# Tung-I/Dual-awareness-Attention-for-Few-shot-Object-Detection

Hardware: AMD Instinct MI355X
Metric: query-images/sec (res50, way=2, shot=3, bs=4 per GPU, train-mode forward) (higher is better)
Workload: dtype f32 (operands, accumulation, results; multiplies as an exact bf16x3 split, six bf16 MFMA products each)

## Files before the change

dual-awareness-attention-for-few-shot-object-detection_amd/csrc/igemm.hip:

```cpp
#include "common.h"
#include "../../include/dana_hip_debug.h"
#include <stdlib.h>
#include <atomic>

namespace {

typedef float f32x16 __attribute__((ext_vector_type(16)));
typedef unsigned int u32x4 __attribute__((ext_vector_type(4)));

struct IgemmParams {
  const float* A;
  const float* Bw;
  float* C;
  const float* scale;
  const float* shift;
  const float* residual;
  const float* mask;
  long ldm;
  int M, N, K;
  int IH, IW, OH, OW, Cin, KH, KW, stride, pad;
  int M0, IH1, IW1, OH1, OW1, pix1;
  float* C1;
  const float* residual1;
  long ldc1, ldr1;
  int lda, ldb;
  long ldc, ldr;
  long batch_a, batch_b, batch_c;
  unsigned a_bytes, b_bytes;
  float alpha;
  int relu;
  int vec_io;
  int vec_ss;
  int tiles_m, tiles_n;
  const float* A2;
  int lda2, IH2, IW2, stride2, K1;
  int IH21, IW21, pix21;
  int bpre;
  const void* Bw2;
  const float* scale2;
  const float* shift2;
  int N2, relu2;
  unsigned a2_bytes;
  int apre, a_rows;
  int res_sample, res_h, res_w, res_oh, res_ow;
  unsigned res_bytes;
  unsigned long long* trace;
};

constexpr int BK = 32;
constexpr int LDS_LD = 36;
constexpr unsigned OOB = 0x80000000u;

__device__ __forceinline__ int xcd_remap(int bid, int nwg) {
  const int q = nwg / 8, r = nwg % 8;
  const int xcd = bid % 8, local = bid / 8;
  return (xcd < r ? xcd * (q + 1) : r * (q + 1) + (xcd - r) * q) + local;
}

__device__ __forceinline__ float4 ldg_b128(__amdgpu_buffer_rsrc_t r, unsigned off) {
  u32x4 v = __builtin_amdgcn_raw_buffer_load_b128(r, (int)off, 0, 0);
  return *(float4*)&v;
}

template <int BM, int BN, int STEM>
__global__ void __launch_bounds__(256, 2) igemm_f32_kernel(IgemmParams p) {
  constexpr int TM = BM / 64, TN = BN / 64;
  constexpr int RA = BM / 32, RB = BN / 32;
  constexpr int CLD = BN + 4;
  extern __shared__ __attribute__((aligned(16))) float smem[];
  float* As = smem;
  float* Bs = smem + 2 * BM * LDS_LD;

  const int tid = threadIdx.x;
  const int lane = tid & 63, wave = tid >> 6;
  const int wm = wave >> 1, wn = wave & 1;
  const int li = lane & 31, lh = lane >> 5;

  const int vid = xcd_remap((int)(blockIdx.z * gridDim.x + blockIdx.x), (int)(gridDim.x * gridDim.z));
  const int zb = vid / (int)gridDim.x;
  const int tile = vid - zb * (int)gridDim.x;
// ... 398 lines not shown
  const int lane = tid & 63, wave = tid >> 6;
  const int wm = wave >> 1, wn = wave & 1;
  const int li = lane & 31, lh = lane >> 5;

  const unsigned long long t_start = p.trace ? __builtin_readcyclecounter() : 0ull;
  const unsigned long long w_start = p.trace ? wall_clock64() : 0ull;
  const int vid = xcd_remap((int)(blockIdx.z * gridDim.x + blockIdx.x), (int)(gridDim.x * gridDim.z));
  const int zb = vid / (int)gridDim.x;
  const int tile = vid - zb * (int)gridDim.x;
  const int tm_idx = tile / p.tiles_n, tn_idx = tile % p.tiles_n;
  const int m0 = tm_idx * BM, n0 = tn_idx * BN;
  const float* Ab = p.A + (long)zb * p.batch_a;
  const float* Bb = p.Bw + (long)zb * p.batch_b;
  float* Cb = p.C + (long)zb * p.batch_c;
  __amdgpu_buffer_rsrc_t ra_src = __builtin_amdgcn_make_buffer_rsrc((void*)Ab, 0, (int)p.a_bytes, 0x00020000);
  const __amdgpu_buffer_rsrc_t rb_src = __builtin_amdgcn_make_buffer_rsrc((void*)Bb, 0, (int)p.b_bytes, 0x00020000);

  int cin_t = STEM ? SBK : p.Cin;
  const int kw_t = STEM ? 2 : p.KW;
  const int kh_t = STEM ? 7 : p.KH;
  const int lda4 = (STEM ? 4 : p.lda) * 4;
  const int kwstep = STEM ? 4 * lda4 : lda4;
  const int c4 = tid & 3;
  const int r0 = tid >> 2;
  const int wcol = ((c4 >> 1) ^ swz(r0)) * 4 + (c4 & 1) * 2;
  const int rcol = (lh ^ swz(li)) * 4;
  const int klim = p.K - c4 * 4;
  constexpr int DEAD = (int)0x80000000;
  unsigned a_off[RA];
  unsigned a_mask[RA];
  int a_dseg[RA];
  unsigned a_off2[RA];
  const bool lin = !STEM && p.KH * p.KW == 1 && p.stride == 1 && p.pad == 0;
#pragma unroll
  for (int j = 0; j < RA; ++j) {
    const int m = m0 + r0 + 64 * j;
    const bool ok = m < p.M;
    const bool s1 = ok && m >= p.M0;
    const int mm = ok ? (s1 ? m - p.M0 : m) : 0;
    if (lin && !p.A2) {
      a_off[j] = (unsigned)(((s1 ? p.pix1 : 0) + mm) * lda4 + c4 * 16);
      a_mask[j] = ok ? 1u : 0u;
      a_dseg[j] = 0;
      a_off2[j] = OOB;
      continue;
    }
    const int IH = s1 ? p.IH1 : p.IH, IW = s1 ? p.IW1 : p.IW, OW = s1 ? p.OW1 : p.OW;
    const int ohw = (s1 ? p.OH1 : p.OH) * OW;
    const int img = mm / ohw, rem = mm - img * ohw;
    const int oh = rem / OW, ow = rem - oh * OW;
    const int ih0 = oh * p.stride - p.pad, iw0 = ow * p.stride - p.pad;
    const int pix = (s1 ? p.pix1 : 0) + (img * IH + ih0) * IW;
    unsigned mask = 0;
    if (STEM) {
      const int lo = ih0 < 0 ? -ih0 : 0, hi = IH - ih0 < 7 ? IH - ih0 : 7;
      const int iwa = iw0 + c4, iwb = iw0 + 4 + c4;
      const unsigned cv = ((iwa >= 0 && iwa < IW) ? 0x1555u : 0u) | ((iwb >= 0 && iwb < IW && c4 < 3) ? 0x2aaau : 0u);
      if (ok && hi > lo) mask = ((1u << (2 * hi)) - (1u << (2 * lo))) & cv;
    } else if (ok) {
      unsigned colbits = 0;
      for (int kw = 0; kw < kw_t; ++kw)
        if (iw0 + kw >= 0 && iw0 + kw < IW) colbits |= 1u << kw;
      for (int kh = 0; kh < kh_t; ++kh)
        if (ih0 + kh >= 0 && ih0 + kh < IH) mask |= colbits << (kh * kw_t);
    }
    a_off[j] = STEM ? (unsigned)((pix + iw0 + c4) * lda4) : (unsigned)((pix + iw0) * lda4 + c4 * 16);
    a_mask[j] = mask;
    a_dseg[j] = s1 ? (p.IW1 - p.IW) * lda4 : 0;
    a_off2[j] = (!STEM && p.A2 && ok)
                    ? (unsigned)(((s1 ? p.pix21 : 0) + ((long)img * (s1 ? p.IH21 : p.IH2) + oh * p.stride2) * (s1 ? p.IW21 : p.IW2) +
                                  ow * p.stride2) * p.lda2 * 4 + c4 * 16)
                    : OOB;
  }
  unsigned b_cur[RB];
  int b_lim[RB];
  int b_lds[RB];
#pragma unroll
  for (int j = 0; j < RB; ++j) {
    if constexpr (BPRE) {
      const int q = (tid + 256 * j < 6 * BN) ? tid + 256 * j : tid;
      const int pl = q / (2 * BN), rem = q - pl * (2 * BN);
      const int row = rem >> 1, half = rem & 1;
      const int n = n0 + row;
      b_cur[j] = (unsigned)((((long)pl * p.N + n) * SBK + half * 8) * 2);
      b_lim[j] = n < p.N ? (p.K + SBK - 1) / SBK * SBK : DEAD;
      b_lds[j] = (pl * BN + row) * SLD + (half ^ swz(row)) * 4;
    } else {
      const int n = n0 + r0 + 64 * j;
      b_cur[j] = (unsigned)((n * p.ldb + c4 * 4) * 4);
      b_lim[j] = n < p.N ? klim : DEAD;
      b_lds[j] = 0;
    }
  }
  const unsigned B_STEP = BPRE ? (unsigned)p.N * 3u * SBK * 2u : SBK * 4;

  float4 ra0[RA], rb0[RB], ra1[RA], rb1[RB];
  int lt_k0 = 0, lt_cin = 0, lt_kh = 0, lt_kw = 0;
  unsigned lt_bit = 1u;
  unsigned a_cur[RA];
  int a_lim[RA];
#pragma unroll
  for (int j = 0; j < RA; ++j) {
    a_cur[j] = a_off[j];
    a_lim[j] = (a_mask[j] & 1u) ? klim : DEAD;
  }
  auto next_tap = [&]() {
    if (lt_cin >= cin_t) {
      lt_cin = 0;
      if (!STEM && p.A2) {
        ra_src = __builtin_amdgcn_make_buffer_rsrc((void*)p.A2, 0, (int)p.a2_bytes, 0x00020000);
        cin_t = 0x7fffffff;
#pragma unroll
        for (int j = 0; j < RA; ++j) {
          a_cur[j] = a_off2[j];
          a_lim[j] = a_off2[j] != OOB ? klim : DEAD;
        }
        return;
      }
// ... 180 lines not shown
            asm volatile("" : "+v"(lb[f][e0]), "+v"(lb[f][e1]));
          } else if constexpr (r == 8) {
            hp[f].x = __builtin_amdgcn_perm(hb[f][1], hb[f][0], 0x07060302u);
            hp[f].y = __builtin_amdgcn_perm(hb[f][3], hb[f][2], 0x07060302u);
            asm volatile("" : "+v"(hp[f].x), "+v"(hp[f].y));
          } else if constexpr (r == 9) {
            mp[f].x = __builtin_amdgcn_perm(mb[f][1], mb[f][0], 0x07060302u);
            mp[f].y = __builtin_amdgcn_perm(mb[f][3], mb[f][2], 0x07060302u);
            asm volatile("" : "+v"(mp[f].x), "+v"(mp[f].y));
          } else if constexpr (r == 10) {
            lp[f].x = __builtin_amdgcn_perm(lb[f][1], lb[f][0], 0x07060302u);
            lp[f].y = __builtin_amdgcn_perm(lb[f][3], lb[f][2], 0x07060302u);
            asm volatile("" : "+v"(lp[f].x), "+v"(lp[f].y));
          } else {
            unsigned* w = f < RA ? aw + 64 * f * SLD : bw + 64 * (f - RA) * SLD;
            constexpr int rows = f < RA ? BM : BN;
            if constexpr (r == 11) {
              *(uint2*)(w + 0 * rows * SLD) = hp[f];
              *(uint2*)(w + 1 * rows * SLD) = mp[f];
            } else {
              *(uint2*)(w + 2 * rows * SLD) = lp[f];
            }
          }
        }
      });
      __builtin_amdgcn_sched_barrier(0);
    });
  };
  const unsigned long long t_loop = p.trace ? __builtin_readcyclecounter() : 0ull;
  for (int t = 0; t < nk; t += 2) {
    k_step(0, fa0, fb0, fa1, fb1, ra0, rb0, ra1, rb1);
    k_step(1, fa1, fb1, fa0, fb0, ra1, rb1, ra0, rb0);
  }
  if constexpr (FUSE || ELDS) __syncthreads();
  const unsigned long long t_loop_end = p.trace ? __builtin_readcyclecounter() : 0ull;

  if constexpr (FUSE) {
    static_assert(BM == 128 && BN == 64 && !STEM && BPRE, "fused tail: 128 x 64 tile over pre-split weights");
    unsigned short* A2 = (unsigned short*)smem;
    unsigned* rtab = (unsigned*)smem + 4 * 3 * BM * 16 * 2 / 4;
    if constexpr (FUSE == 2) {
      if (tid < BM) {
        const int m = m0 + tid;
        unsigned off = OOB;
        if (m < p.M) {
          const int ohw = p.OH * p.OW;
          const int img = m / ohw, rem = m - img * ohw;
          const int oh = rem / p.OW, ow = rem - oh * p.OW;
          off = (unsigned)((((long)img * p.IH + oh * p.stride) * p.IW + ow * p.stride) * p.ldr * 4);
        }
        rtab[tid] = off;
      }
    }
    {
      const int nn = wn * 32 + li;
      const float sc1 = p.scale ? p.scale[nn] : 1.f, sh1 = p.shift ? p.shift[nn] : 0.f;
      const int ks = nn >> 4, kk = nn & 15;
#pragma unroll
      for (int i = 0; i < TM; ++i)
#pragma unroll
        for (int r = 0; r < 16; ++r) {
          const int row = wm * (BM / 2) + i * 32 + (r & 3) + 8 * (r >> 2) + 4 * lh;
          float v = acc[i][0][r] * sc1 + sh1;
          if (p.relu) v = fmaxf(v, 0.f);
          const unsigned hb = __float_as_uint(v) & 0xffff0000u;
          const float r1 = v - __uint_as_float(hb);
          const unsigned mb = __float_as_uint(r1) & 0xffff0000u;
          const unsigned lb = __float_as_uint(r1 - __uint_as_float(mb));
// ... 269 lines not shown
      const bool s1 = m >= p.M0;
      float* cp = s1 ? p.C1 + (long)(m - p.M0) * p.ldc1 + n : Cb + (long)m * p.ldc + n;
      const float* rp = s1 ? p.residual1 + (long)(m - p.M0) * p.ldr1 + n : p.residual + (long)m * p.ldr + n;
      for (int t = 0; t < 4; ++t)
        if ((n + t) < p.N) {
          float x = Cs[rr * CLD + ec + t] * sc[t] + sh[t];
          if (p.residual) x += rp[t];
          if (p.relu) x = fmaxf(x, 0.f);
          if (p.mask && !(p.mask[(long)m * p.ldm + n + t] > 0.f)) x = 0.f;
          cp[t] = x;
        }
    }
  }
  if (p.trace && tid == 0) {
    unsigned long long* tr = p.trace + ((long)blockIdx.z * gridDim.x + blockIdx.x) * 8;
    tr[0] = t_start;
    tr[1] = t_loop;
    tr[2] = t_loop_end;
    tr[3] = __builtin_readcyclecounter();
    tr[4] = (unsigned long long)__builtin_amdgcn_s_getreg((31 << 11) | 4) | ((unsigned long long)__builtin_amdgcn_s_getreg((31 << 11) | 20) << 32);
    tr[5] = wall_clock64();
    tr[6] = w_start;
    tr[7] = 0;
  }
}

template <int BM, int BN, int STEM, int BPRE = 0, int FUSE = 0, int ELDS = 0, int RSMP = 0>
__global__ void __launch_bounds__(256, 2) igemm_split_kernel(IgemmParams p) {
  igemm_split_body<BM, BN, STEM, BPRE, FUSE, ELDS, RSMP>(p);
}
template <int STEM, int BPRE, int ELDS, int RSMP = 0>
__global__ void __launch_bounds__(256, 1) __attribute__((amdgpu_num_vgpr(192))) igemm_split_kernel_128(IgemmParams p) {
  igemm_split_body<128, 128, STEM, BPRE, 0, ELDS, RSMP>(p);
}

template <int BN, int NST, int APRE, int DF = 0>
__global__ void __launch_bounds__(256, NST == 2 ? 3 : (NST == 3 ? 2 : 1)) igemm_dma_kernel(IgemmParams p) {
  static_assert(APRE || NST == 2, "fp32 activation rows: two stages");
  static_assert(!DF || (APRE && NST >= 3), "two fragment sets: planes x planes, three or more stages");
  constexpr int BM = 128, TM = 2, TN = BN / 64;
  constexpr int STAGE_B = 3 * (BM + BN) * 32;
  constexpr int NPB = 3 * BN / 32, PB = (NPB + 3) / 4;
  constexpr int NDMA = (APRE ? 3 : 0) + PB;
  constexpr int AHEAD = NST == 2 ? 2 : NST - 1;
  constexpr int RA = BM / 64;
  extern __shared__ __attribute__((aligned(16))) float smem[];
  const int tid = threadIdx.x;
  const int lane = tid & 63, wave = __builtin_amdgcn_readfirstlane(tid >> 6);
  const int wm = wave >> 1, wn = wave & 1;
  const int li = lane & 31, lh = lane >> 5;
  const unsigned long long t_start = p.trace ? __builtin_readcyclecounter() : 0ull;
  const unsigned long long w_start = p.trace ? wall_clock64() : 0ull;
  const int vid = xcd_remap((int)(blockIdx.z * gridDim.x + blockIdx.x), (int)(gridDim.x * gridDim.z));
  const int zb = vid / (int)gridDim.x;
  const int tile = vid - zb * (int)gridDim.x;
  const int tm_idx = tile / p.tiles_n, tn_idx = tile % p.tiles_n;
  const int m0 = tm_idx * BM, n0 = tn_idx * BN;
  float* Cb = p.C + (long)zb * p.batch_c;
  __amdgpu_buffer_rsrc_t ra_src =
      __builtin_amdgcn_make_buffer_rsrc((void*)(p.A + (long)zb * p.batch_a), 0, (int)p.a_bytes, 0x00020000);
  const __amdgpu_buffer_rsrc_t rb_src =
      __builtin_amdgcn_make_buffer_rsrc((void*)(p.Bw + (long)zb * p.batch_b), 0, (int)p.b_bytes, 0x00020000);
  const int nk = (p.K + SBK - 1) / SBK;

  const int prow = lane >> 1, phalf = (lane & 1) ^ ((lane >> 4) & 1);
  const int arow = m0 + 32 * wave + prow;
// ... 354 lines not shown
  igemm_f32_kernel<BM, BN, STEM><<<grid, 256, lds, s>>>(p);
  return 0;
}

template <int BM, int BN, int STEM = 0, int BPRE = 0, int FUSE = 0, int ELDS = 0, int RSMP = 0>
int launch_split(const IgemmParams& p0, int batch, hipStream_t s) {
  if constexpr (BPRE == 0 && FUSE == 0) {
    if (p0.bpre) return launch_split<BM, BN, STEM, 1, 0, ELDS, RSMP>(p0, batch, s);
  }
  if constexpr (ELDS == 0 && FUSE == 0 && RSMP == 0) {
    if (epilogue_mode_cell().load(std::memory_order_relaxed)) return launch_split<BM, BN, STEM, BPRE, 0, 1>(p0, batch, s);
  }
  g_last_form.store(form_code(BM * BN >= 128 * 128 ? DANA_IGEMM_FAMILY_SPLIT_128 : DANA_IGEMM_FAMILY_SPLIT, BM, BN, STEM, BPRE, FUSE ? 1 : 0,
                              ELDS, 0, 0, 0), std::memory_order_relaxed);
  IgemmParams p = p0;
  p.tiles_m = (p.M + BM - 1) / BM;
  p.tiles_n = (p.N + BN - 1) / BN;
  size_t lds = (size_t)2 * 3 * (BM + BN) * SLD * sizeof(unsigned);
  const size_t lds_c = (size_t)BM * (BN + 4) * sizeof(float);
  if (lds_c > lds && ELDS) lds = lds_c;
  if (FUSE && lds < (size_t)4 * 3 * BM * 16 * 2) lds = (size_t)4 * 3 * BM * 16 * 2;
  if (FUSE == 2 || RSMP) lds += (size_t)BM * 4;
  dim3 grid(p.tiles_m * p.tiles_n, 1, batch);
  static DeviceOnce attr;
  if constexpr (BM * BN >= 128 * 128) {
    attr.once([&] { return hipFuncSetAttribute((const void*)igemm_split_kernel_128<STEM, BPRE, ELDS, RSMP>, hipFuncAttributeMaxDynamicSharedMemorySize,
                                (int)lds); });
    igemm_split_kernel_128<STEM, BPRE, ELDS, RSMP><<<grid, 256, lds, s>>>(p);
  } else {
    attr.once([&] { return hipFuncSetAttribute((const void*)igemm_split_kernel<BM, BN, STEM, BPRE, FUSE, ELDS, RSMP>,
                                hipFuncAttributeMaxDynamicSharedMemorySize, (int)lds); });
    igemm_split_kernel<BM, BN, STEM, BPRE, FUSE, ELDS, RSMP><<<grid, 256, lds, s>>>(p);
  }
  return 0;
}

template <int BN, int NST, int APRE, int DF = 0>
int launch_dma(const IgemmParams& p0, int batch, hipStream_t s) {
  g_last_form.store(form_code(DANA_IGEMM_FAMILY_DMA, 128, BN, 0, 1, 0, 0, NST, APRE, DF), std::memory_order_relaxed);
  IgemmParams p = p0;
  p.tiles_m = (p.M + 127) / 128;
  p.tiles_n = (p.N + BN - 1) / BN;
  const size_t lds = (size_t)NST * 3 * (128 + BN) * 32;
  static DeviceOnce attr;
  attr.once([&] { return hipFuncSetAttribute((const void*)igemm_dma_kernel<BN, NST, APRE, DF>, hipFuncAttributeMaxDynamicSharedMemorySize, (int)lds); });
  dim3 grid(p.tiles_m * p.tiles_n, 1, batch);
  igemm_dma_kernel<BN, NST, APRE, DF><<<grid, 256, lds, s>>>(p);
  return 0;
}

std::atomic<int>& mfma_mode_cell() {
  static std::atomic<int> cell(getenv("DANA_MFMA_SPLIT") ? atoi(getenv("DANA_MFMA_SPLIT")) : 1);
  return cell;
}
int env_choice(const char* name, std::initializer_list<int> allowed) {
  const char* e = getenv(name);
  if (!e || !*e) return -1;
  const int v = atoi(e);
  for (int a : allowed)
    if (a == v) return v;
  fprintf(stderr, "libdana_hip: %s=%s is not one of the accepted values; ignored\n", name, e);
  return -1;
}
int dma_kernel_env() {
  static const int v = env_choice("DANA_DMA_KERNEL", {0, 1, 2});
  return v;
// ... 214 lines not shown
  p.ldc = out0_stride > 0 ? out0_stride : cout;
  p.ldr = res0_stride > 0 ? res0_stride : cout;
  p.ldc1 = out1_stride > 0 ? out1_stride : cout;
  p.ldr1 = res1_stride > 0 ? res1_stride : cout;
  DANA_CHECK_ARG(((uintptr_t)input & 15) == 0 && ((uintptr_t)weight & 15) == 0,
                 "%s: input/weight must be 16-byte aligned", who);
  if (res_sample > 0 && res0) {
    DANA_CHECK_ARG(batch1 == 0 && !mask && res_h > 0 && res_w > 0 && (res_h - 1) / res_sample + 1 == p.OH &&
                       (res_w - 1) / res_sample + 1 == p.OW,
                   "%s: sampled residual: one segment, no mask, and (res_h - 1) / res_sample + 1 x (res_w - 1) / res_sample + 1 must be the output map", who);
    const long res_bytes = (long)batch0 * res_h * res_w * p.ldr * 4;
    DANA_CHECK_ARG(res_bytes < (long)OOB, "%s: residual span >= 2 GiB; split the batch", who);
    p.res_sample = res_sample;
    p.res_h = res_h;
    p.res_w = res_w;
    p.res_oh = p.OH;
    p.res_ow = p.OW;
    p.res_bytes = (unsigned)res_bytes;
  }
  const int rc = run(p, 1, stem, (hipStream_t)stream);
  DANA_CHECK_ARG(rc == 0, "%s: a sampled residual needs the split kernel's register epilogue at a 64 x 64 or 128 x 128 tile "
                          "(dana_set_mfma_mode(1), dana_set_epilogue_mode(0), cout > 64, at most 32 taps)", who);
  DANA_CHECK_LAUNCH(who);
  return DANA_OK;
}

int dana_conv2d_nhwc(const float* input, const float* weight, float* output, const float* scale,
                     const float* shift, const float* residual, int batch, int in_h, int in_w, int cin,
                     int cout, int kh, int kw, int stride, int pad, long in_pix_stride, long out_pix_stride,
                     long res_pix_stride, int flags, dana_stream_t stream) {
  return conv2d_impl("dana_conv2d_nhwc", input, weight, output, nullptr, scale, shift, residual, nullptr, batch, in_h,
                     in_w, 0, 0, 0, cin, cout, kh, kw, stride, pad, in_pix_stride, out_pix_stride, 0, res_pix_stride,
                     0, flags, stream);
}

int dana_conv2d_nhwc_sampled_res(const float* input, const float* weight, float* output, const float* scale,
                                 const float* shift, const float* residual, int batch, int in_h, int in_w, int cin,
                                 int cout, int kh, int kw, int stride, int pad, long in_pix_stride, long out_pix_stride,
                                 long res_pix_stride, int res_h, int res_w, int res_sample, int flags, dana_stream_t stream) {
  const char* who = "dana_conv2d_nhwc_sampled_res";
  DANA_CHECK_ARG(residual && res_sample >= 1 && res_sample <= 2, "%s: needs a residual and res_sample 1 or 2", who);
  return conv2d_impl(who, input, weight, output, nullptr, scale, shift, residual, nullptr, batch, in_h, in_w, 0, 0, 0, cin,
                     cout, kh, kw, stride, pad, in_pix_stride, out_pix_stride, 0, res_pix_stride, 0, flags, stream, nullptr, 0,
                     res_h, res_w, res_sample);
}

int dana_conv2d_nhwc_masked(const float* input, const float* weight, float* output, const float* scale,
                            const float* shift, const float* residual, const float* mask_act, int batch, int in_h,
                            int in_w, int cin, int cout, int kh, int kw, int stride, int pad, long in_pix_stride,
                            long out_pix_stride, long res_pix_stride, long mask_pix_stride, int flags,
                            dana_stream_t stream) {
  return conv2d_impl("dana_conv2d_nhwc_masked", input, weight, output, nullptr, scale, shift, residual, nullptr, batch,
                     in_h, in_w, 0, 0, 0, cin, cout, kh, kw, stride, pad, in_pix_stride, out_pix_stride, 0,
                     res_pix_stride, 0, flags, stream, mask_act, mask_pix_stride);
}

static int tail_impl(const char* who, const float* input, const float* w2_split, const float* scale2, const float* shift2,
                     const float* w3_split, const float* scale3, const float* shift3, const float* residual,
                     float* output, int batch, int h, int w, int cin, int cmid, int cout, long in_pix_stride,
                     long out_pix_stride, long res_pix_stride, int stride, int flags, dana_stream_t stream) {
  DANA_CHECK_ARG(batch >= 0 && h > 0 && w > 0 && (stride == 1 || stride == 2), "%s: bad shape (stride 1 or 2)", who);
  if (batch == 0) return DANA_OK;
  DANA_CHECK_ARG(input && w2_split && w3_split && output, "%s: null pointer", who);
  DANA_CHECK_ARG(cmid == 64 && cin % SBK == 0 && cin > 0 && cout % 64 == 0 && cout > 0,
                 "%s: needs 64 middle channels, cin %% 16 == 0, cout %% 64 == 0", who);
  DANA_CHECK_ARG(dana_get_mfma_mode() != 0, "%s: split kernel only (dana_set_mfma_mode != 0)", who);
// ... 258 lines not shown
```

dual-awareness-attention-for-few-shot-object-detection_amd/dana.py:

```python
import contextlib
import math
import time
from types import SimpleNamespace

import numpy as np
import torch
import torch.nn as nn
import torch.nn.functional as F

from . import ops
from .config import cfg
from . import targets as T
from .cached_inputs import (BankEpisode, ClassSweep, QueryBank, QueryBatch, SupportBank, SupportCache,
                            check_cached_forward, query_batch_size, query_device, read_inputs, resolve_bank_episode,
                            resolve_query_batch, resolve_shot_views)


class Bottleneck(nn.Module):
    expansion = 4

    def __init__(self, inplanes, planes, stride=1, downsample=None):
        super().__init__()
        self.conv1 = nn.Conv2d(inplanes, planes, kernel_size=1, stride=stride, bias=False)
        self.bn1 = nn.BatchNorm2d(planes)
# ... 75 lines not shown
    def forward(fctx, anchor, model, l1, l2, l3, l4):
        fctx.model = model
        fctx.saved = model._ctx
        return l1.clone(), l2.clone(), l3.clone(), l4.clone()

    @staticmethod
    def backward(fctx, g1, g2, g3, g4):
        from . import backward as BW
        ctx = fctx.saved
        if ctx is None or ctx.get("consumed"):
            raise RuntimeError("the saved activations of this training forward were already consumed by a backward pass "
                               "(each forward can be differentiated once; run the forward again)")
        gs = [torch.zeros((), device=fctx.model._grad_anchor.device) if g is None else g.reshape(()) for g in (g1, g2, g3, g4)]
        fctx.saved = None
        BW.model_backward(fctx.model, torch.stack(gs), ctx=ctx)
        return None, None, None, None, None, None


_HERE = contextlib.nullcontext()

ATTENTION_LEVELS = ("ba", "rpn", "roi")


def _on(stream):
    return _HERE if stream is None else ops.on_stream(stream)


def _rows(t, row):
    return t[row:] if row and t is not None else t


class DAnARCNN(nn.Module):
    trim_strided_seams = True

    def __init__(self, classes, attention_type="concat", rpn_reduce_dim=256, rcnn_reduce_dim=256, gamma=0.1,
                 semantic_enhance=False, num_layers=50, pretrained=False, num_way=2, num_shot=5, pos_encoding=True):
        super().__init__()
        if attention_type not in ("concat", "product"):
            raise ValueError("attention_type must be 'concat' or 'product' (dana.py:70-77)")
        self.model_path = "data/pretrained_model/resnet50_caffe.pth"
        self.dout_base_model = 1024
        self.pretrained = pretrained
        self.classes = classes
        self.n_classes = len(classes)
        self.n_way = num_way
        self.n_shot = num_shot
        self.attention_type = attention_type
        self.channel_gamma = gamma
        self.unary_gamma = 0.1
        self.semantic_enhance = semantic_enhance
        self.rpn_reduce_dim = rpn_reduce_dim
        self.rcnn_reduce_dim = rcnn_reduce_dim
        self.pos_encoding = pos_encoding
        self.pool_feat_dim = 1024
        self.rcnn_dim = 64
        self.use_winograd = True
        self.winograd_tile = 4
        self.winograd_min_cin = 128
        self.presplit_weights = True
        self.merge_trunk = False
        self.merge_from = 0
        self.fold_roi_pe = True
        self.fold_roi_attn = True
        self.prefetch_dgrad = "layer4"
        self.rpn_side_role = "wgrad"
        self.nms_inclusive = False
# ... 273 lines not shown
        return [(_rows(o, s[2]), cols) for s in segs]

    def _conv(self, segs, osegs, x, c, relu, merged=False, res=None, res_stride=0, outs=None, in_stride=0, keep=None,
              alloc=None, stem=False):
        cin, cout, k, sd, pd = 4 if stem else c["cin"], c["cout"], c["k"], c["stride"], c["pad"]
        u = c.get("u")
        wino = u is not None and res is None and (not merged or (u.size(0) == 36 and outs is None))
        b = (c.get("us") or u) if wino else self._b(c)
        dest = self._dest(osegs, cout, outs, alloc, x.device)
        if merged:
            (n0, (h0, w0), _, _), (n1, (h1, w1), _, _) = segs
            (o0, s0), (o1, s1) = dest
            if wino:
                ops.conv3x3_winograd_dual(x, n0, h0, w0, n1, h1, w1, cin, b, cout, scale=c["scale"], shift=c["shift"],
                                          relu=relu, out=o0)
            else:
                ops.conv2d_nhwc_dual(x, n0, h0, w0, n1, h1, w1, cin, b, cout, k, k, sd, pd, scale=c["scale"],
                                     shift=c["shift"], res0=res, res1=_rows(res, osegs[1][2]), relu=relu, in_stride=in_stride,
                                     out0=o0, out1=o1, out0_stride=s0, out1_stride=s1, res0_stride=res_stride,
                                     res1_stride=res_stride, stem=stem)
            return o0
        for i, ((n, (h, w), row, st), (o, ld)) in enumerate(zip(segs, dest)):
            with _on(st):
                if wino:
                    ops.conv3x3_winograd(_rows(x, row), n, h, w, cin, b, cout, scale=c["scale"], shift=c["shift"], relu=relu,
                                         in_stride=in_stride, out=o, out_stride=ld,
                                         keep_v=keep[i] if keep is not None else None)
                else:
                    ops.conv2d_nhwc(_rows(x, row), n, h, w, cin, b, cout, k, k, sd, pd, scale=c["scale"], shift=c["shift"],
                                    residual=_rows(res, osegs[i][2]), relu=relu, in_stride=in_stride, out=o, out_stride=ld,
                                    res_stride=res_stride, stem=stem)
        return dest[0][0]

    def _stem(self, segs, ims, c, merged, alloc):
        csegs = self._grid(segs, lambda h, w: ((h - 1) // 2 + 1, (w - 1) // 2 + 1))
        psegs = self._grid(csegs, ops.maxpool_out_size)
        dev = ims[0].device
        x4, xs, xp = (self._dest(g, cols, None, alloc, dev) for g, cols in ((segs, 4), (csegs, 64), (psegs, 64)))
        for g in ([slice(None)] if merged else [slice(i, i + 1) for i in range(len(segs))]):
            for im, (o, _), (_, _, _, st) in zip(ims[g], x4[g], segs[g]):
                with _on(st):
                    ops.nchw_to_nhwc(im, cpad=4, out=o)
            self._conv(segs[g], csegs[g], x4[0][0], c, True, merged, outs=xs[g], stem=True)
            for (n, (h, w), row, st), (o, _) in zip(csegs[g], xp[g]):
                with _on(st):
                    ops.maxpool3x3s2_ceil(_rows(xs[0][0], row), n, h, w, 64, out=o)
        return xp[0][0], psegs

    def _can_trim(self, bp, nbp):
        n1, nds = nbp["c1"], nbp["ds"]
        if nds is None or any((c["k"], c["stride"], c["pad"]) != (1, 2, 0) for c in (n1, nds)):
            return False
        c1, c2, c3 = bp["c1"], bp["c2"], bp["c3"]
        if bp["ds"] is not None or c1["stride"] != 1 or (c2["k"], c2["stride"], c2["pad"]) != (3, 1, 1) or ops.get_mfma_mode() != 1:
            return False
        if c2["cout"] == 64 and c2.get("u") is None and c2["ws"] is not None and c3["ws"] is not None:
            return True
        u = c2.get("u")
        return (u is not None and u.size(0) == 36 and c3["cout"] > 64 and c3["cout"] % 128 == 0
                and ops.get_epilogue_mode() == 0)

    def _block(self, segs, x, bp, merged=False, outs=None, in_stride=0, saves=None, key=None, alloc=None, save_m=None,
               trim=False, pre=False):
        if merged and in_stride:
            raise ValueError("a merged block reads dense rows")
        if saves is not None and saves[0] is None:
            saves = None
        c1, c2, c3, ds = bp["c1"], bp["c2"], bp["c3"], bp["ds"]
        dev, cout, sd = x.device, c3["cout"], 1 if pre else c1["stride"]
        if pre:
# ... 86 lines not shown
    def _rcnn_base(self, im, plan, out_stride=0, out_buf=None, save=None, save_from=1):
        x, ((_, (h, w), _, _),), _ = self._drain(self._trunk_gen(
            [im], plan, outs=[(out_buf, out_stride)], saves=[save], save_from=save_from))
        return x, h, w

    def _trunk_gen(self, ims, plan, outs=((None, 0),), saves=None, side=None, merge_from=None, save_m=None, save_from=1):
        two, dev = len(ims) > 1, ims[0].device
        alloc = None
        if two:
            main = ops.cur_stream()
            if side == main:
                side = None

            def alloc(rows, cols):
                t = torch.empty((rows, cols), dtype=torch.float32, device=dev)
                if side is not None:
                    t.record_stream(side)
                    ev = torch.cuda.Event()
                    ev.record(main)
                    side.wait_event(ev)
                return t

        def join(segs):
            if side is not None:
                main.wait_event(ops.record_event(side))
            return [(n, hw, row, None) for n, hw, row, _ in segs]

        merged = two and merge_from <= 0
        segs, row = [], 0
        for i, im in enumerate(ims):
            n, _, H, W = im.shape
            segs.append((n, (H, W), row, side if i and not merged else None))
            row += n * H * W
        x, segs = self._stem(segs, ims, plan["stem"], merged, alloc)
        yield
        nl = len(plan["layers"])
        nosave, pre = saves is None or all(s is None for s in saves), False
        stall = getattr(self, "_debug_stall", None) if two else None
        for li, layer in enumerate(plan["layers"]):
            if two and not merged and li >= merge_from:
                segs, merged = join(segs), True
            for bi, bp in enumerate(layer):
                last = (li == nl - 1) and (bi == len(layer) - 1)
                if stall is not None and not merged and li == stall[0]:
                    torch.cuda._sleep(int(stall[1]))
                trim = (self.trim_strided_seams and not last and bi == len(layer) - 1 and li + 1 < nl and not merged
                        and not (two and li + 1 >= merge_from) and (nosave or li + 1 < save_from)
                        and self._can_trim(bp, plan["layers"][li + 1][0]))
                x, segs, dest = self._block(segs, x, bp, merged, outs=outs if last and outs[0][1] else None,
                                            saves=saves if li >= save_from else None, key="RCNN_base.%d.%d" % (4 + li, bi), alloc=alloc,
                                            save_m=save_m, trim=trim, pre=pre)
                pre = trim
                if not last:
                    yield
        if two and not merged:
            segs = join(segs)
        return x, segs, dest

    @staticmethod
    def _feat_size(H, W):
        h, w = (H + 6 - 7) // 2 + 1, (W + 6 - 7) // 2 + 1
        h, w = ops.maxpool_out_size(h, w)
        for _ in range(2):
            h, w = (h - 1) // 2 + 1, (w - 1) // 2 + 1
        return h, w

    def _check_support_map(self, sh_, sw_):
        if (sh_, sw_) != (20, 20):
            if not self.generalised_support or sh_ % 7 or sw_ % 7:
                raise RuntimeError("support images must be 320x320 (20x20 stride-16 map), as the reference hard-codes "
# ... 857 lines not shown
```

dual-awareness-attention-for-few-shot-object-detection_amd/ops.py:

```python
import collections
import contextlib
import ctypes
import time as _time

import torch

from ._lib import lib, DanaError

HOST_WAIT = [0.0]

NCHW, NHWC = 0, 1
EPI_RELU, CONV_STEM7, W_SPLIT3, A_SPLIT3 = 1, 2, 256, 512

PROFILE = None
PROF_ROLE = None


def _prof_begin():
    if PROFILE is None:
        return None
    e = torch.cuda.Event(enable_timing=True)
    e.record()
    return e

# ... 571 lines not shown
    lib().call("dana_plain_rcnn_loss", _p(_chk(scores, "scores")), _p(labels), _p(_chk(bbox_pred.contiguous(), "bbox_pred")),
               _p(_chk(bbox_targets.contiguous(), "bbox_targets")), _p(_chk(inside_ws.contiguous(), "inside_ws")),
               _p(_chk(outside_ws.contiguous(), "outside_ws")), n, c, float(sigma), _p(out),
               _p(seeds[0]) if seeds else None, _p(seeds[1]) if seeds else None, _stream())
    return out, seeds


def conv2d_nhwc(x, batch, in_h, in_w, cin, weight, cout, kh, kw, stride, pad, scale=None, shift=None,
                residual=None, relu=False, in_stride=0, out=None, out_stride=0, res_stride=0, stem=False, res_hw=None,
                res_sample=0):
    _chk(x, "x")
    wp, wfl = _wf(weight)
    oh = (in_h + 2 * pad - kh) // stride + 1
    ow = (in_w + 2 * pad - kw) // stride + 1
    if out is None:
        out = torch.empty((batch * oh * ow, cout), dtype=torch.float32, device=x.device)
        out_stride = cout
    flags = (EPI_RELU if relu else 0) | (CONV_STEM7 if stem else 0) | wfl
    e0 = _prof_begin()
    if res_sample:
        lib().call("dana_conv2d_nhwc_sampled_res", _p(x), wp, _p(out), _p(scale), _p(shift), _p(_chk(residual, "residual")),
                   batch, in_h, in_w, cin, cout, kh, kw, stride, pad, in_stride, out_stride, res_stride, res_hw[0], res_hw[1],
                   int(res_sample), flags, _stream())
    else:
        lib().call("dana_conv2d_nhwc", _p(x), wp, _p(out), _p(scale), _p(shift), _p(residual), batch, in_h,
                   in_w, cin, cout, kh, kw, stride, pad, in_stride, out_stride, res_stride, flags, _stream())
    _prof_end(e0, ("conv%dx%d M=%d N=%d K=%d s%d", (kh, kw, batch * oh * ow, cout, kh * kw * cin, stride)),
              2.0 * batch * oh * ow * cout * kh * kw * (3 if stem else cin),
              4.0 * (batch * in_h * in_w * cin // (stride * stride if kh == 1 else 1) + cout * kh * kw * cin
                     + batch * oh * ow * cout * (2 if residual is not None else 1)))
    return out, oh, ow


def bottleneck_tail(x, batch, h, w, cin, w2, scale2, shift2, w3, scale3, shift3, cout, residual=None, relu=True, in_stride=0,
                    out=None, out_stride=0, res_stride=0, stride=1):
    _chk(x, "x")
    if not (isinstance(w2, W3) and isinstance(w3, W3)):
        raise TypeError("bottleneck_tail: both weights must be split planes (ops.split_weight)")
    oh, ow = (h - 1) // stride + 1, (w - 1) // stride + 1
    if out is None:
        out = torch.empty((batch * oh * ow, cout), dtype=torch.float32, device=x.device)
        out_stride = cout
    e0 = _prof_begin()
    if stride == 1:
        lib().call("dana_bottleneck_tail_nhwc", _p(x), _p(w2.t), _p(scale2), _p(shift2), _p(w3.t), _p(scale3), _p(shift3),
                   _p(residual), _p(out), batch, h, w, cin, 64, cout, in_stride, out_stride, res_stride,
                   EPI_RELU if relu else 0, _stream())
    else:
        lib().call("dana_bottleneck_tail_strided_nhwc", _p(x), _p(w2.t), _p(scale2), _p(shift2), _p(w3.t), _p(scale3),
                   _p(shift3), _p(residual), _p(out), batch, h, w, cin, 64, cout, in_stride, out_stride, res_stride,
                   int(stride), EPI_RELU if relu else 0, _stream())
    m = batch * oh * ow
    _prof_end(e0, ("conv3x3+1x1 M=%d N=%d K=%d+64 s%d", (m, cout, 9 * cin, stride)), 2.0 * m * 64 * (9 * cin + cout),
              4.0 * (batch * h * w * cin + 64 * 9 * cin + 64 * cout + m * cout * (2 if residual is not None else 1)))
    return out, oh, ow


def conv2d_nhwc_dual(x, n0, h0, w0, n1, h1, w1, cin, weight, cout, kh, kw, stride, pad, scale=None, shift=None,
                     res0=None, res1=None, relu=False, in_stride=0, out0=None, out1=None, out0_stride=0,
                     out1_stride=0, res0_stride=0, res1_stride=0, stem=False):
    _chk(x, "x")
    wp, wfl = _wf(weight)
    oh0, ow0 = (h0 + 2 * pad - kh) // stride + 1, (w0 + 2 * pad - kw) // stride + 1
    oh1, ow1 = (h1 + 2 * pad - kh) // stride + 1, (w1 + 2 * pad - kw) // stride + 1
    m0, m1 = n0 * oh0 * ow0, n1 * oh1 * ow1
    if out0 is None:
# ... 1006 lines not shown
```

include/dana_hip.h:

```cpp
#ifndef DANA_HIP_H
#define DANA_HIP_H
#include <stddef.h>
#include <stdint.h>

#ifdef __cplusplus
extern "C" {
#endif

typedef void* dana_stream_t;

#define DANA_LAYOUT_NCHW 0
#define DANA_LAYOUT_NHWC 1

#define DANA_EPI_RELU 1
#define DANA_CONV_STEM7 2
#define DANA_W_SPLIT3 256
#define DANA_A_SPLIT3 512

const char* dana_last_error(void);
int dana_abi_version(void);

int dana_set_mfma_mode(int mode);
int dana_get_mfma_mode(void);

// ... 71 lines not shown
                       const int* index, int n_sets, int B, dana_stream_t stream);
int dana_gather_shot_blocks(const void* src_ptrs, const void* dst_ptrs, const long long* rows, const long long* block_bytes,
                            int n_tensors, const int* index, const int* view, float* w, int n_sets, int shot, int m, int P,
                            dana_stream_t stream);
int dana_bank_gather_episode(const float* map_pe, const float* pool_pe, const int* index, int n_bank, int B, int way,
                             int shot, int map_rows, int pool_rows, int channels, float* s_pe, float* sp_pe,
                             dana_stream_t stream);
int dana_qbank_gather(const float* maps, const int* index, int n_bank, int B, int rows, int channels, float* out, int ld_out,
                      dana_stream_t stream);

int dana_attn_softmax_unary_sweep(const float* scores, float* out, const float* unary, int B, int C, long hw,
                                  long unary_stride, int nseg, int length, long ld_in, long ld_out, int kpad,
                                  float unary_gamma, float out_scale, dana_stream_t stream);
int dana_attn_softmax_unary_sweep_w(const float* scores, float* out, const float* unary, int B, int C, long hw,
                                    long unary_stride, int nseg, int length, long ld_in, long ld_out, int kpad,
                                    float unary_gamma, const float* seg_scale, long scale_stride, dana_stream_t stream);
int dana_repeat_rows_grouped(const float* src, float* dst, long rows, int cols, long ld_src, long ld_dst, int group,
                             long n_blocks, dana_stream_t stream);
int dana_mul_rows_grouped(float* y, const float* x, long rows, int channels, long ld_y, long ld_x, int group,
                          long n_blocks, dana_stream_t stream);
int dana_meta_class_head(const float* fc7, const float* vec, const float* weight, const float* bias, const float* rois,
                         const float* bbox_pred, float* cls_prob, float* rois_out, float* bbox_out, int B, int C, int R,
                         int K, dana_stream_t stream);
int dana_roi_align_forward_nhwc_grouped(const float* input, const float* rois, float* output, int batch, int channels,
                                        int height, int width, int num_rois, float spatial_scale, int pooled,
                                        int sampling_ratio, long in_pix_stride, long out_pix_stride, float* output2,
                                        const float* add2, long out2_pix_stride, int group, dana_stream_t stream);


int dana_conv2d_nhwc(const float* input, const float* weight, float* output, const float* scale,
                     const float* shift, const float* residual, int batch, int in_h, int in_w, int cin,
                     int cout, int kh, int kw, int stride, int pad, long in_pix_stride, long out_pix_stride,
                     long res_pix_stride, int flags, dana_stream_t stream);

int dana_conv2d_nhwc_masked(const float* input, const float* weight, float* output, const float* scale,
                            const float* shift, const float* residual, const float* mask_act, int batch, int in_h,
                            int in_w, int cin, int cout, int kh, int kw, int stride, int pad, long in_pix_stride,
                            long out_pix_stride, long res_pix_stride, long mask_pix_stride, int flags,
                            dana_stream_t stream);
int dana_bottleneck_tail_nhwc(const float* input, const float* w2_split, const float* scale2, const float* shift2,
                              const float* w3_split, const float* scale3, const float* shift3, const float* residual,
                              float* output, int batch, int h, int w, int cin, int cmid, int cout, long in_pix_stride,
                              long out_pix_stride, long res_pix_stride, int flags, dana_stream_t stream);
int dana_bottleneck_tail_strided_nhwc(const float* input, const float* w2_split, const float* scale2, const float* shift2,
                                      const float* w3_split, const float* scale3, const float* shift3,
                                      const float* residual, float* output, int batch, int h, int w, int cin, int cmid,
                                      int cout, long in_pix_stride, long out_pix_stride, long res_pix_stride, int stride,
                                      int flags, dana_stream_t stream);
int dana_conv2d_nhwc_sampled_res(const float* input, const float* weight, float* output, const float* scale,
                                 const float* shift, const float* residual, int batch, int in_h, int in_w, int cin,
                                 int cout, int kh, int kw, int stride, int pad, long in_pix_stride, long out_pix_stride,
                                 long res_pix_stride, int res_h, int res_w, int res_sample, int flags, dana_stream_t stream);

int dana_conv2d_nhwc_dual(const float* input, const float* weight, float* out0, float* out1, const float* scale,
                          const float* shift, const float* res0, const float* res1, int batch0, int h0, int w0,
                          int batch1, int h1, int w1, int cin, int cout, int kh, int kw, int stride, int pad,
                          long in_pix_stride, long out0_stride, long out1_stride, long res0_stride,
                          long res1_stride, int flags, dana_stream_t stream);

int dana_winograd_filter_transform(const float* w_packed, float* u, int cout, int cin, dana_stream_t stream);
size_t dana_conv3x3_winograd_workspace_bytes(int batch, int h, int w, int cin, int cout);
int dana_conv3x3_winograd_nhwc(const float* input, const float* u, float* output, const float* scale,
                               const float* shift, int batch, int h, int w, int cin, int cout, long in_pix_stride,
                               long out_pix_stride, int flags, void* workspace, size_t workspace_bytes,
                               dana_stream_t stream);
int dana_conv3x3_winograd_nhwc_masked(const float* input, const float* u, float* output, const float* scale,
// ... 325 lines not shown
```

include/dana_hip_debug.h:

```cpp
#ifndef DANA_HIP_DEBUG_H
#define DANA_HIP_DEBUG_H
#include "dana_hip.h"

#ifdef __cplusplus
extern "C" {
#endif

int dana_debug_force_tile(int tile);
int dana_set_epilogue_mode(int mode);
int dana_get_epilogue_mode(void);
int dana_debug_set_dma_kernel(int v);
int dana_debug_get_dma_kernel(void);
int dana_debug_set_pp_stages(int v);
int dana_debug_get_pp_stages(void);
#define DANA_IGEMM_FAMILY_F32 1
#define DANA_IGEMM_FAMILY_SPLIT 2
#define DANA_IGEMM_FAMILY_SPLIT_128 3
#define DANA_IGEMM_FAMILY_DMA 4
int dana_debug_last_igemm_form(void);
int dana_set_igemm_trace(unsigned long long* buffer);
int dana_set_sort_mode(int mode);

int dana_debug_stream_create_cumask(const unsigned int* mask, int mask_words, int n_xcd, dana_stream_t* stream_out);
int dana_debug_stream_destroy(dana_stream_t stream);

size_t dana_debug_radix_sort_workspace_bytes(long n);
int dana_debug_radix_sort_pairs(const unsigned long long* keys_in, const int* vals_in, unsigned long long* keys_out,
                                int* vals_out, long n, int key_bits, void* workspace, size_t workspace_bytes,
                                dana_stream_t stream);

#ifdef __cplusplus
}
#endif
#endif
```

Before: 736.7.

## Fuse the 7x7 stem conv with the 3x3/s2 max-pool in one tiled kernel

Adds a stem kernel variant in which each 256-row tile covers a 15x17 patch of conv outputs (with halo) for a 7x8 block of pooled outputs. The tile applies scale, shift and ReLU in registers, stages the result in LDS and writes only the max-pooled values. This removes the write and re-read of the full-resolution stem activation and one separate pool launch. In exchange, halo rows are recomputed in overlapping tiles and some tile rows are idle (255 of 256 used). It is used only on the non-merged path when no stem activations need saving.

```diff
diff --git a/dual-awareness-attention-for-few-shot-object-detection_amd/csrc/igemm.hip b/dual-awareness-attention-for-few-shot-object-detection_amd/csrc/igemm.hip
--- a/dual-awareness-attention-for-few-shot-object-detection_amd/csrc/igemm.hip
+++ b/dual-awareness-attention-for-few-shot-object-detection_amd/csrc/igemm.hip
@@ -45,7 +45,12 @@
   int res_sample, res_h, res_w, res_oh, res_ow;
   unsigned res_bytes;
   unsigned long long* trace;
+  int pool_oh, pool_ow, pool_tiles_h, pool_tiles_w;
 };
+
+constexpr int POOL_PH = 7, POOL_PW = 8;
+constexpr int POOL_CH = 2 * POOL_PH + 1, POOL_CW = 2 * POOL_PW + 1;
+constexpr int POOL_LD = 72;
 
 constexpr int BK = 32;
 constexpr int LDS_LD = 36;
@@ -510,11 +515,29 @@
   int a_dseg[RA];
   unsigned a_off2[RA];
   const bool lin = !STEM && p.KH * p.KW == 1 && p.stride == 1 && p.pad == 0;
+  int pt_img = 0, pt_ph = 0, pt_pw = 0;
+  if constexpr (STEM == 2) {
+    const int per_img = p.pool_tiles_h * p.pool_tiles_w;
+    pt_img = tile / per_img;
+    const int rem = tile - pt_img * per_img;
+    pt_ph = rem / p.pool_tiles_w;
+    pt_pw = rem - pt_ph * p.pool_tiles_w;
+  }
+  const int pt_oh0 = 2 * POOL_PH * pt_ph, pt_ow0 = 2 * POOL_PW * pt_pw;
 #pragma unroll
   for (int j = 0; j < RA; ++j) {
     const int m = m0 + r0 + 64 * j;
-    const bool ok = m < p.M;
-    const bool s1 = ok && m >= p.M0;
+    int p_oh = 0, p_ow = 0;
+    bool p_ok = true;
+    if constexpr (STEM == 2) {
+      const int r = r0 + 64 * j;
+      const int loh = r / POOL_CW;
+      p_oh = pt_oh0 + loh;
+      p_ow = pt_ow0 + (r - loh * POOL_CW);
+      p_ok = loh < POOL_CH && p_oh < p.OH && p_ow < p.OW;
+    }
+    const bool ok = STEM == 2 ? p_ok : m < p.M;
+    const bool s1 = STEM != 2 && ok && m >= p.M0;
     const int mm = ok ? (s1 ? m - p.M0 : m) : 0;
     if (lin && !p.A2) {
       a_off[j] = (unsigned)(((s1 ? p.pix1 : 0) + mm) * lda4 + c4 * 16);
@@ -525,8 +548,8 @@
     }
     const int IH = s1 ? p.IH1 : p.IH, IW = s1 ? p.IW1 : p.IW, OW = s1 ? p.OW1 : p.OW;
     const int ohw = (s1 ? p.OH1 : p.OH) * OW;
-    const int img = mm / ohw, rem = mm - img * ohw;
-    const int oh = rem / OW, ow = rem - oh * OW;
+    const int img = STEM == 2 ? pt_img : mm / ohw, rem = mm - img * ohw;
+    const int oh = STEM == 2 ? (p_ok ? p_oh : 0) : rem / OW, ow = STEM == 2 ? (p_ok ? p_ow : 0) : rem - oh * OW;
     const int ih0 = oh * p.stride - p.pad, iw0 = ow * p.stride - p.pad;
     const int pix = (s1 ? p.pix1 : 0) + (img * IH + ih0) * IW;
     unsigned mask = 0;
@@ -561,7 +584,7 @@
       const int row = rem >> 1, half = rem & 1;
       const int n = n0 + row;
       b_cur[j] = (unsigned)((((long)pl * p.N + n) * SBK + half * 8) * 2);
-      b_lim[j] = n < p.N ? (p.K + SBK - 1) / SBK * SBK : DEAD;
+      b_lim[j] = (STEM == 2 || n < p.N) ? (p.K + SBK - 1) / SBK * SBK : DEAD;
       b_lds[j] = (pl * BN + row) * SLD + (half ^ swz(row)) * 4;
     } else {
       const int n = n0 + r0 + 64 * j;
@@ -808,8 +831,53 @@
     k_step(0, fa0, fb0, fa1, fb1, ra0, rb0, ra1, rb1);
     k_step(1, fa1, fb1, fa0, fb0, ra1, rb1, ra0, rb0);
   }
-  if constexpr (FUSE || ELDS) __syncthreads();
+  if constexpr (FUSE || ELDS || STEM == 2) __syncthreads();
   const unsigned long long t_loop_end = p.trace ? __builtin_readcyclecounter() : 0ull;
+
+  if constexpr (STEM == 2) {
+    static_assert(BM == 256 && BN == 64 && BPRE && !FUSE && !ELDS && !RSMP, "stem + pool: one 256 x 64 patch tile");
+    float* Ps = smem;
+    {
+      const int nn = wn * 32 + li;
+      const float scv = (p.scale ? p.scale[nn] : 1.f) * p.alpha, shv = p.shift ? p.shift[nn] : 0.f;
+      float* pw = Ps + (wm * (BM / 2) + 4 * lh) * POOL_LD + nn;
+#pragma unroll
+      for (int i = 0; i < TM; ++i)
+#pragma unroll
+        for (int r = 0; r < 16; ++r) {
+          float v = acc[i][0][r] * scv + shv;
+          if (p.relu) v = fmaxf(v, 0.f);
+          pw[(i * 32 + (r & 3) + 8 * (r >> 2)) * POOL_LD] = v;
+        }
+    }
+    __syncthreads();
+    const int pc4 = (tid & 15) * 4;
+    const int oh_left = p.OH - pt_oh0, ow_left = p.OW - pt_ow0;
+#pragma unroll
+    for (int pass = 0; pass < (POOL_PH * POOL_PW + 15) / 16; ++pass) {
+      const int pp = (tid >> 4) + 16 * pass;
+      const int lpy = pp / POOL_PW, lpx = pp - lpy * POOL_PW;
+      const int py = POOL_PH * pt_ph + lpy, px = POOL_PW * pt_pw + lpx;
+      if (lpy < POOL_PH && py < p.pool_oh && px < p.pool_ow) {
+        float4 mx = make_float4(-3.402823466e+38f, -3.402823466e+38f, -3.402823466e+38f, -3.402823466e+38f);
+#pragma unroll
+        for (int dh = 0; dh < 3; ++dh) {
+          if (2 * lpy + dh >= oh_left) break;
+#pragma unroll
+          for (int dw = 0; dw < 3; ++dw) {
+            if (2 * lpx + dw >= ow_left) break;
+            const float4 v = *(const float4*)(Ps + ((2 * lpy + dh) * POOL_CW + 2 * lpx + dw) * POOL_LD + pc4);
+            mx.x = fmaxf(mx.x, v.x);
+            mx.y = fmaxf(mx.y, v.y);
+            mx.z = fmaxf(mx.z, v.z);
+            mx.w = fmaxf(mx.w, v.w);
+          }
+        }
+        *(float4*)(Cb + (((long)pt_img * p.pool_oh + py) * p.pool_ow + px) * p.ldc + pc4) = mx;
+      }
+    }
+    return;
+  }
 
   if constexpr (FUSE) {
     static_assert(BM == 128 && BN == 64 && !STEM && BPRE, "fused tail: 128 x 64 tile over pre-split weights");
@@ -1145,6 +1213,9 @@
 template <int STEM, int BPRE, int ELDS, int RSMP = 0>
 __global__ void __launch_bounds__(256, 1) __attribute__((amdgpu_num_vgpr(192))) igemm_split_kernel_128(IgemmParams p) {
   igemm_split_body<128, 128, STEM, BPRE, 0, ELDS, RSMP>(p);
+}
+__global__ void __launch_bounds__(256, 1) __attribute__((amdgpu_num_vgpr(192))) igemm_stem_pool_kernel(IgemmParams p) {
+  igemm_split_body<256, 64, 2, 1>(p);
 }
 
 template <int BN, int NST, int APRE, int DF = 0>
@@ -1565,6 +1636,20 @@
                                 hipFuncAttributeMaxDynamicSharedMemorySize, (int)lds); });
     igemm_split_kernel<BM, BN, STEM, BPRE, FUSE, ELDS, RSMP><<<grid, 256, lds, s>>>(p);
   }
+  return 0;
+}
+
+int launch_stem_pool(const IgemmParams& p0, hipStream_t s) {
+  g_last_form.store(form_code(DANA_IGEMM_FAMILY_SPLIT, 0, 64, 1, 1, 0, 0, 0, 0, 0) | DANA_IGEMM_FORM_POOL, std::memory_order_relaxed);
+  IgemmParams p = p0;
+  p.tiles_n = 1;
+  size_t lds = (size_t)2 * 3 * (256 + 64) * SLD * sizeof(unsigned);
+  const size_t lds_p = (size_t)256 * POOL_LD * sizeof(float);
+  if (lds_p > lds) lds = lds_p;
+  static DeviceOnce attr;
+  attr.once([&] { return hipFuncSetAttribute((const void*)igemm_stem_pool_kernel, hipFuncAttributeMaxDynamicSharedMemorySize, (int)lds); });
+  dim3 grid(p.tiles_m, 1, 1);
+  igemm_stem_pool_kernel<<<grid, 256, lds, s>>>(p);
   return 0;
 }
 
@@ -1845,6 +1930,66 @@
   return conv2d_impl("dana_conv2d_nhwc", input, weight, output, nullptr, scale, shift, residual, nullptr, batch, in_h,
                      in_w, 0, 0, 0, cin, cout, kh, kw, stride, pad, in_pix_stride, out_pix_stride, 0, res_pix_stride,
                      0, flags, stream);
+}
+
+int dana_stem_conv_pool_nhwc(const float* input, const float* weight_split, float* output, const float* scale,
+                             const float* shift, int batch, int in_h, int in_w, int cin, int cout, long out_pix_stride,
+                             int flags, dana_stream_t stream) {
+  const char* who = "dana_stem_conv_pool_nhwc";
+  DANA_CHECK_ARG(batch >= 0 && in_h > 0 && in_w > 0, "%s: bad shape", who);
+  DANA_CHECK_ARG(cin == 4 && cout == 64, "%s: the 7x7 stem over NHWC4 with 64 filters only (cin=%d cout=%d)", who, cin, cout);
+  DANA_CHECK_ARG((flags & DANA_W_SPLIT3) != 0, "%s: the filters must be dana_split_weight planes (DANA_W_SPLIT3)", who);
+  DANA_CHECK_ARG(mfma_mode_cell().load(std::memory_order_relaxed) != 0 && epilogue_mode_cell().load(std::memory_order_relaxed) == 0,
+                 "%s: needs the split kernel's register epilogue (dana_set_mfma_mode(1), dana_set_epilogue_mode(0))", who);
+  if (batch == 0) return DANA_OK;
+  DANA_CHECK_ARG(input && weight_split && output, "%s: null pointer", who);
+  const long ldc = out_pix_stride > 0 ? out_pix_stride : cout;
+  DANA_CHECK_ARG(ldc >= cout && ldc % 4 == 0 && ((uintptr_t)output & 15) == 0 && ((uintptr_t)input & 15) == 0 &&
+                     ((uintptr_t)weight_split & 15) == 0,
+                 "%s: input / weights / output rows must be 16-byte aligned, out_pix_stride >= cout", who);
+  IgemmParams p;
+  memset(&p, 0, sizeof(p));
+  p.A = input;
+  p.Bw = weight_split;
+  p.C = p.C1 = output;
+  p.scale = scale;
+  p.shift = shift;
+  p.IH = p.IH1 = in_h;
+  p.IW = p.IW1 = in_w;
+  p.OH = p.OH1 = (in_h - 1) / 2 + 1;
+  p.OW = p.OW1 = (in_w - 1) / 2 + 1;
+  DANA_CHECK_ARG(p.OH >= 3 && p.OW >= 3, "%s: the conv map must hold one pooling window", who);
+  p.pool_oh = (p.OH - 3 + 1) / 2 + 1;
+  p.pool_ow = (p.OW - 3 + 1) / 2 + 1;
+  if ((p.pool_oh - 1) * 2 >= p.OH) --p.pool_oh;
+  if ((p.pool_ow - 1) * 2 >= p.OW) --p.pool_ow;
+  p.pool_tiles_h = (p.pool_oh + POOL_PH - 1) / POOL_PH;
+  p.pool_tiles_w = (p.pool_ow + POOL_PW - 1) / POOL_PW;
+  const long tiles = (long)batch * p.pool_tiles_h * p.pool_tiles_w;
+  const long a_bytes = (long)batch * in_h * in_w * 16, b_bytes = (long)3 * cout * 224 * 2;
+  DANA_CHECK_ARG(a_bytes < (long)OOB && tiles * 256 < (long)OOB, "%s: input span >= 2 GiB; split the batch", who);
+  p.tiles_m = (int)tiles;
+  p.M = p.M0 = (int)(tiles * 256);
+  p.N = cout;
+  p.KH = p.KW = 7;
+  p.stride = 2;
+  p.pad = 3;
+  p.Cin = 4;
+  p.K = 7 * 32;
+  p.lda = 4;
+  p.ldb = p.K;
+  p.bpre = 1;
+  p.a_bytes = (unsigned)a_bytes;
+  p.b_bytes = (unsigned)b_bytes;
+  p.ldc = p.ldc1 = ldc;
+  p.ldr = p.ldr1 = cout;
+  p.alpha = 1.f;
+  p.relu = (flags & DANA_EPI_RELU) ? 1 : 0;
+  p.ldm = cout;
+  p.trace = nullptr;
+  launch_stem_pool(p, (hipStream_t)stream);
+  DANA_CHECK_LAUNCH(who);
+  return DANA_OK;
 }
 
 int dana_conv2d_nhwc_sampled_res(const float* input, const float* weight, float* output, const float* scale,
diff --git a/dual-awareness-attention-for-few-shot-object-detection_amd/dana.py b/dual-awareness-attention-for-few-shot-object-detection_amd/dana.py
--- a/dual-awareness-attention-for-few-shot-object-detection_amd/dana.py
+++ b/dual-awareness-attention-for-few-shot-object-detection_amd/dana.py
@@ -131,6 +131,7 @@
 
 class DAnARCNN(nn.Module):
     trim_strided_seams = True
+    fuse_stem_pool = True
 
     def __init__(self, classes, attention_type="concat", rpn_reduce_dim=256, rcnn_reduce_dim=256, gamma=0.1,
                  semantic_enhance=False, num_layers=50, pretrained=False, num_way=2, num_shot=5, pos_encoding=True):
@@ -470,10 +471,18 @@
                                     res_stride=res_stride, stem=stem)
         return dest[0][0]
 
-    def _stem(self, segs, ims, c, merged, alloc):
+    def _stem(self, segs, ims, c, merged, alloc, fuse=False):
         csegs = self._grid(segs, lambda h, w: ((h - 1) // 2 + 1, (w - 1) // 2 + 1))
         psegs = self._grid(csegs, ops.maxpool_out_size)
         dev = ims[0].device
+        if fuse and not merged:
+            x4, xp = (self._dest(g, cols, None, alloc, dev) for g, cols in ((segs, 4), (psegs, 64)))
+            for im, (o4, _), (n, (h, w), row, st), (o, ld) in zip(ims, x4, segs, xp):
+                with _on(st):
+                    ops.nchw_to_nhwc(im, cpad=4, out=o4)
+                    ops.stem_conv_pool(o4, n, h, w, 4, c["ws"], c["cout"], scale=c["scale"], shift=c["shift"], relu=True,
+                                       out=o, out_stride=ld)
+            return xp[0][0], psegs
         x4, xs, xp = (self._dest(g, cols, None, alloc, dev) for g, cols in ((segs, 4), (csegs, 64), (psegs, 64)))
         for g in ([slice(None)] if merged else [slice(i, i + 1) for i in range(len(segs))]):
             for im, (o, _), (_, _, _, st) in zip(ims[g], x4[g], segs[g]):
@@ -626,10 +635,12 @@
             n, _, H, W = im.shape
             segs.append((n, (H, W), row, side if i and not merged else None))
             row += n * H * W
-        x, segs = self._stem(segs, ims, plan["stem"], merged, alloc)
+        nosave, pre = saves is None or all(s is None for s in saves), False
+        fuse_stem = (self.fuse_stem_pool and not merged and (nosave or save_from >= len(plan["layers"]))
+                     and plan["stem"]["ws"] is not None and ops.get_mfma_mode() != 0 and ops.get_epilogue_mode() == 0)
+        x, segs = self._stem(segs, ims, plan["stem"], merged, alloc, fuse=fuse_stem)
         yield
         nl = len(plan["layers"])
-        nosave, pre = saves is None or all(s is None for s in saves), False
         stall = getattr(self, "_debug_stall", None) if two else None
         for li, layer in enumerate(plan["layers"]):
             if two and not merged and li >= merge_from:
diff --git a/dual-awareness-attention-for-few-shot-object-detection_amd/ops.py b/dual-awareness-attention-for-few-shot-object-detection_amd/ops.py
--- a/dual-awareness-attention-for-few-shot-object-detection_amd/ops.py
+++ b/dual-awareness-attention-for-few-shot-object-detection_amd/ops.py
@@ -627,6 +627,29 @@
     return out, oh, ow
 
 
+STEM_POOL_PATCH = (7, 8)
+
+
+def stem_conv_pool(x, batch, in_h, in_w, cin, weight, cout, scale=None, shift=None, relu=True, out=None, out_stride=0):
+    _chk(x, "x")
+    if not isinstance(weight, W3):
+        raise TypeError("stem_conv_pool: the weight must be split planes (ops.split_weight)")
+    oh, ow = (in_h - 1) // 2 + 1, (in_w - 1) // 2 + 1
+    ph, pw = maxpool_out_size(oh, ow)
+    if out is None:
+        out = torch.empty((batch * ph * pw, cout), dtype=torch.float32, device=x.device)
+        out_stride = cout
+    e0 = _prof_begin()
+    lib().call("dana_stem_conv_pool_nhwc", _p(x), _p(weight.t), _p(out), _p(scale), _p(shift), batch, in_h, in_w, cin, cout,
+               out_stride, (EPI_RELU if relu else 0) | W_SPLIT3, _stream())
+    tiles = batch * (-(-ph // STEM_POOL_PATCH[0])) * (-(-pw // STEM_POOL_PATCH[1]))
+    _prof_end(e0, ("conv7x7 M=%d N=%d K=%d +pool s%d", (batch * oh * ow, cout, 49 * cin, 2)),
+              2.0 * batch * oh * ow * cout * 49 * 3,
+              4.0 * (batch * in_h * in_w * cin + cout * 49 * cin + batch * ph * pw * cout),
+              executed=2.0 * tiles * 256 * cout * 49 * 3)
+    return out, ph, pw
+
+
 def bottleneck_tail(x, batch, h, w, cin, w2, scale2, shift2, w3, scale3, shift3, cout, residual=None, relu=True, in_stride=0,
                     out=None, out_stride=0, res_stride=0, stride=1):
     _chk(x, "x")
diff --git a/include/dana_hip.h b/include/dana_hip.h
--- a/include/dana_hip.h
+++ b/include/dana_hip.h
@@ -127,6 +127,10 @@
                      const float* shift, const float* residual, int batch, int in_h, int in_w, int cin,
                      int cout, int kh, int kw, int stride, int pad, long in_pix_stride, long out_pix_stride,
                      long res_pix_stride, int flags, dana_stream_t stream);
+
+int dana_stem_conv_pool_nhwc(const float* input, const float* weight_split, float* output, const float* scale,
+                             const float* shift, int batch, int in_h, int in_w, int cin, int cout, long out_pix_stride,
+                             int flags, dana_stream_t stream);
 
 int dana_conv2d_nhwc_masked(const float* input, const float* weight, float* output, const float* scale,
                             const float* shift, const float* residual, const float* mask_act, int batch, int in_h,
diff --git a/include/dana_hip_debug.h b/include/dana_hip_debug.h
--- a/include/dana_hip_debug.h
+++ b/include/dana_hip_debug.h
@@ -13,6 +13,7 @@
 int dana_debug_get_dma_kernel(void);
 int dana_debug_set_pp_stages(int v);
 int dana_debug_get_pp_stages(void);
+#define DANA_IGEMM_FORM_POOL (1 << 18)
 #define DANA_IGEMM_FAMILY_F32 1
 #define DANA_IGEMM_FAMILY_SPLIT 2
 #define DANA_IGEMM_FAMILY_SPLIT_128 3
```

Measured after the change: 739.8, median of 4. About the same (+0.4%).
